# mbzuai-oryx/Video-LLaVA

Hardware: NVIDIA H100
Metric: videos/sec (100-frame CLIP encode + 7B 32-tok decode) (higher is better)
Workload: dtype bf16

## Files before the change

include/vcl.h:

```cpp
#ifndef VCL_H_
#define VCL_H_

#include <stddef.h>
#include <stdint.h>

#ifdef __cplusplus
extern "C" {
#endif

#define VCL_VERSION 1

#define VCL_DTYPE_F16 0
#define VCL_DTYPE_BF16 1

#define VCL_PIXELS_BF16_NCHW 0
#define VCL_PIXELS_U8_NHWC 1

#define VCL_WEIGHTS_BF16 0
#define VCL_WEIGHTS_FP8_E4M3 1

#define VCL_PROJ_LINEAR 0
#define VCL_PROJ_MLP2X_GELU 1

typedef struct vcl_handle vcl_handle;
// ... 110 lines not shown
#define VCL_LOGPROBS_MAX 20
int vcl_llm_set_logprobs(vcl_handle* h, int n, const int32_t* clips_host, const int32_t* top_n_host, void* stream);

int vcl_llm_read_logprobs(vcl_handle* h, int entry, int first_pos, int count, int32_t* ids_out, float* lp_out,
                          void* stream);

#define VCL_BEAM_MAX 8
typedef struct vcl_beam_record {
  float score;
  int32_t beam;
  int32_t token;
} vcl_beam_record;
int vcl_llm_beam_start(vcl_handle* h, const int64_t* ids, const void* video_feats, const int32_t* vid_start,
                       const int32_t* n_pad_host, int B, int S, int num_beams, int n_new, int eos_token,
                       void* records_out, int32_t* picks_out, void* stream);
int vcl_llm_beam_decode(vcl_handle* h, int n_steps, void* records_out, int32_t* picks_out, void* stream);

int vcl_llm_set_block_table(vcl_handle* h, const int32_t* table_host, void* stream);

int vcl_kv_block_copy(vcl_handle* h, int block, int write, void* buf, void* stream);

int vcl_llm_score(vcl_handle* h, const int64_t* ids, const void* video_feats, const int32_t* vid_start,
                  const int32_t* n_pad_host, int B, int S, const int64_t* labels, void* logits_out, float* nll_out,
                  float* loss_out, void* stream);

long long vcl_launch_count(void);

int vcl_op_gemm(const void* A, int64_t lda, const void* W, int64_t ldw, void* C, int64_t ldc,
                const void* bias, const void* residual, int64_t ldr, int M, int N, int K, int act,
                int block_n, void* stream);
int vcl_op_gemm_ex(const void* A, int64_t lda, const void* W, int64_t ldw, void* C, int64_t ldc,
                   const void* bias, const void* residual, int64_t ldr, int M, int N, int K, int act,
                   int block_n, int cluster, void* stream);
int vcl_op_cross_entropy(const void* logits, int64_t ld, const int64_t* labels, int rows, int V,
                         float* nll_out, float* loss_out, void* stream);
int vcl_op_sample(const float* logits, int64_t ld, int B, int V, const float* temperature_host,
                  const int32_t* top_k_host, const uint64_t* seed_host, const int32_t* counter_host, int32_t* tok_out,
                  void* stream);
int vcl_op_sample_logprobs(const float* logits, int64_t ld, int B, int V, const float* temperature_host,
                           const int32_t* top_k_host, const uint64_t* seed_host, const int32_t* counter_host,
                           const int32_t* top_n_host, int32_t* tok_out, int32_t* ids_out, float* lp_out,
                           void* stream);
int vcl_op_sample_ex(const float* logits, int64_t ld, int B, int V, const float* temperature_host,
                     const int32_t* top_k_host, const uint64_t* seed_host, const int32_t* counter_host,
                     const float* top_p_host, const float* repetition_penalty_host, uint32_t* token_sets,
                     const int32_t* top_n_host, int32_t* tok_out, int32_t* ids_out, float* lp_out, void* stream);
int vcl_op_beam_select(const float* logits, int64_t ld, int B, int num_beams, int V, const float* scores, int eos_token,
                       int last_step, void* records_out, int32_t* picks_out, void* stream);
int vcl_op_layernorm(const void* x, void* y, const void* w, const void* b, int rows, int D, float eps,
                     void* stream);
int vcl_op_rmsnorm(const void* x, void* y, const void* w, int rows, int D, float eps, void* stream);
int vcl_op_attention(const void* q, const void* k, const void* v, void* o, int B, int S, int H,
                     int head_dim, float scale, int causal, void* stream);
int vcl_op_attention_vit(const void* qkv, void* out, int n_frames, int S, int H, void* stream);
int vcl_kv_cache_copy(vcl_handle* h, int layer, int write, void* k, void* v, void* stream);
int vcl_op_decode_attention(const void* q, int64_t q_ld, const void* k, const void* v, void* o, int B, int H,
                            int s_max, int kv_len, const int32_t* pos_dev, const int32_t* n_pad, float scale,
                            int o_xwin, void* stream);
int vcl_op_attention_cached(const void* q, int64_t q_ld, const void* k, const void* v, void* o, int B, int H,
                            int s_max, int start_pos, int S, const int32_t* n_pad_host, void* stream);
int vcl_op_attention_packed(const void* q, int64_t q_ld, const void* k, const void* v, void* o, int H, int s_max,
                            int n_slots, int n, const int32_t* slots_host, const int32_t* start_host,
                            const int32_t* len_host, const int32_t* flash_host, const int32_t* table_host,
                            int table_row, int n_blocks, int64_t blk, void* stream);
int vcl_op_gemv(const void* x, const void* W, void* out, const void* res, const void* norm_w,
                float eps, int B, int N, int K, void* stream);
// ... 9 lines not shown
```

video-llava_b200/csrc/gemm_tc.cu:

```cuda
#include "common.cuh"
#include "kernels.h"

#include <cudaTypedefs.h>

namespace vcl {

template <int BLOCK_N>
struct GemmCfg {
  static constexpr int BLOCK_M = 128;
  static constexpr int BLOCK_K = 64;
  static constexpr int A_BYTES = BLOCK_M * BLOCK_K * 2;
  static constexpr int B_BYTES = BLOCK_N * BLOCK_K * 2;
  static constexpr int STAGE_BYTES = A_BYTES + B_BYTES;
  static constexpr int OUT_PITCH = BLOCK_N * 2 + 16;
  static constexpr int OUT_BYTES = BLOCK_M * OUT_PITCH;
  static constexpr int BAR_BYTES = 256;
  static constexpr int STAGES = (BLOCK_N == 256) ? 3 : (BLOCK_N == 128 ? 5 : 8);
  static constexpr int SMEM_BYTES = STAGES * STAGE_BYTES + BAR_BYTES + OUT_BYTES + 1024;
  static_assert((2 * STAGES + 4) * 8 <= BAR_BYTES, "barrier area");
  static_assert(SMEM_BYTES <= 227 * 1024, "shared memory");
};

__device__ __forceinline__ float act_gelu_erf(float x) {
  x = bf16r(x);
// ... 108 lines not shown
      }
    }
#pragma unroll (ACT == ACT_ROPE ? 1 : RES_INFLIGHT)
    for (int u = 0; u < RES_INFLIGHT; ++u) {
      const int r = r0 + u * RSTEP;
      if (r >= rows) break;
      const int grow = row_base + r;
      uint4 val = *reinterpret_cast<const uint4*>(stg + r * Cfg::OUT_PITCH + c * 16);
      bf16* dst = C + (long long)grow * ldc + col;
      if constexpr (ACT == ACT_ROPE) {
        const int gh = col >> 7, d = col & 127;
        const int which = gh / rp.H, head = gh - which * rp.H;
        if (which != 0) {
          int gb, col_c;
          if (rp.pack != nullptr) {
            const int2 sp = __ldg(reinterpret_cast<const int2*>(pack_row(rp.pack, grow)));
            gb = __ldg(pack_slot(rp.pack) + sp.x); col_c = sp.y;
          } else {
            gb = grow / rp.S; col_c = rp.start_pos + grow - gb * rp.S;
          }
          dst = (which == 1 ? rp.kcache : rp.vcache) + d +
                (rp.pages.table != nullptr ? kv_paged_off(rp.pages, gb, head, col_c)
                                           : (((long long)gb * rp.H + head) * rp.s_max + col_c) * 128);
        }
      } else if (RES && residual != nullptr) {
        val.x = bf16x2_add(val.x, rr[u].x); val.y = bf16x2_add(val.y, rr[u].y);
        val.z = bf16x2_add(val.z, rr[u].z); val.w = bf16x2_add(val.w, rr[u].w);
      }
      *reinterpret_cast<uint4*>(dst) = val;
    }
  }
}

template <int BLOCK_N, int ACT, int CL>
__global__ void __launch_bounds__(384, 1)
gemm_bf16_tn_kernel(const __grid_constant__ CUtensorMap tmap_a,
                    const __grid_constant__ CUtensorMap tmap_b, bf16* C, long long ldc,
                    const bf16* __restrict__ bias, const bf16* residual, long long ldr, int M,
                    int N, int K, const RopeEpilogue rope) {
  using Cfg = GemmCfg<BLOCK_N>;
  constexpr int STAGES = Cfg::STAGES;

  extern __shared__ uint8_t smem_raw[];
  const uint32_t raw_addr = smem_u32(smem_raw);
  const uint32_t pad = ((raw_addr + 1023u) & ~1023u) - raw_addr;
  uint8_t* smem = smem_raw + pad;
  const uint32_t smem_base = raw_addr + pad;

  const uint32_t bar_base = smem_base + STAGES * Cfg::STAGE_BYTES;
  auto full_bar = [&](int s) { return bar_base + 8u * s; };
  auto empty_bar = [&](int s) { return bar_base + 8u * (STAGES + s); };
  auto staged_bar = [&](int cw) { return bar_base + 8u * (2 * STAGES + cw); };
  auto drained_bar = [&](int cw) { return bar_base + 8u * (2 * STAGES + 2 + cw); };
  uint8_t* stage_out = smem + STAGES * Cfg::STAGE_BYTES + Cfg::BAR_BYTES;

  const int wg = threadIdx.x >> 7;

  if (threadIdx.x == 0) {
    tma_prefetch_desc(&tmap_a);
    tma_prefetch_desc(&tmap_b);
    for (int s = 0; s < STAGES; ++s) {
      mbar_init(full_bar(s), 1);
      mbar_init(empty_bar(s), 2 * CL);
    }
    for (int cw = 0; cw < 2; ++cw) {
      mbar_init(staged_bar(cw), 128);
      mbar_init(drained_bar(cw), STORE_THREADS);
    }
    mbar_fence_init();
  }
  __syncthreads();
  if (CL > 1) cluster_sync_all();

  const int num_m = (M + Cfg::BLOCK_M - 1) / Cfg::BLOCK_M;
  const int num_n = (N + BLOCK_N - 1) / BLOCK_N;
  const int num_k = (K + Cfg::BLOCK_K - 1) / Cfg::BLOCK_K;
  const int cta_rank = CL > 1 ? (int)cluster_ctarank() : 0;
  const int cluster_id = blockIdx.x / CL, n_clusters = gridDim.x / CL;
  const int num_tiles = ((num_m + CL - 1) / CL) * num_n;
  constexpr uint16_t MC_MASK = (uint16_t)((1u << CL) - 1u);
  constexpr int B_SLICE_ROWS = BLOCK_N / CL;

  if (wg == 0) {
    setmaxnreg_dec<56>();
    if (threadIdx.x == 0) {
      int stage = 0;
      uint32_t phase = 0;
      for (int tile = cluster_id; tile < num_tiles; tile += n_clusters) {
        const int m_blk = (tile / num_n) * CL + cta_rank, n_blk = tile % num_n;
        for (int kb = 0; kb < num_k; ++kb) {
          mbar_wait(empty_bar(stage), phase ^ 1u);
          mbar_arrive_expect_tx(full_bar(stage), Cfg::STAGE_BYTES);
          const uint32_t a_dst = smem_base + stage * Cfg::STAGE_BYTES;
          tma_load_2d(a_dst, &tmap_a, full_bar(stage), kb * Cfg::BLOCK_K, m_blk * Cfg::BLOCK_M);
          if (CL == 1) {
            tma_load_2d(a_dst + Cfg::A_BYTES, &tmap_b, full_bar(stage), kb * Cfg::BLOCK_K, n_blk * BLOCK_N);
          } else {
            tma_load_2d_mc(a_dst + Cfg::A_BYTES + cta_rank * B_SLICE_ROWS * 128, &tmap_b,
                           full_bar(stage), kb * Cfg::BLOCK_K, n_blk * BLOCK_N + cta_rank * B_SLICE_ROWS,
                           MC_MASK);
          }
          if (++stage == STAGES) { stage = 0; phase ^= 1u; }
        }
      }
    } else if (threadIdx.x >= 32) {
      const int t = threadIdx.x - 32;
      uint32_t phase = 0;
      for (int tile = cluster_id; tile < num_tiles; tile += n_clusters) {
        const int m_blk = (tile / num_n) * CL + cta_rank, n_blk = tile % num_n;
#pragma unroll 1
        for (int cw = 0; cw < 2; ++cw) {
          mbar_wait(staged_bar(cw), phase);
          gemm_epilogue_store<BLOCK_N, ACT>(stage_out + cw * 64 * Cfg::OUT_PITCH, t, m_blk * Cfg::BLOCK_M + cw * 64,
                                            n_blk, C, ldc, residual, ldr, M, N, rope);
          mbar_arrive(drained_bar(cw));
        }
        phase ^= 1u;
      }
    }
  } else {
    setmaxnreg_inc<224>();
    const int cw = wg - 1;
    const int t = threadIdx.x & 127, lane = threadIdx.x & 31, wq = t >> 5;
    uint8_t* stg = stage_out + cw * 64 * Cfg::OUT_PITCH;
    auto release = [&](int s) {
      if (t == 0) {
        if (CL == 1) {
          mbar_arrive(empty_bar(s));
        } else {
#pragma unroll
          for (int r = 0; r < CL; ++r) mbar_arrive_cluster(mapa_cluster(empty_bar(s), (uint32_t)r));
        }
      }
    };
    float acc[BLOCK_N / 2];
    int stage = 0;
    uint32_t phase = 0, out_phase = 0;
    for (int tile = cluster_id; tile < num_tiles; tile += n_clusters) {
      const int m_blk = (tile / num_n) * CL + cta_rank, n_blk = tile % num_n;
      int prev = -1;
      for (int kb = 0; kb < num_k; ++kb) {
        mbar_wait(full_bar(stage), phase);
        const uint32_t a_addr = smem_base + stage * Cfg::STAGE_BYTES;
        const uint64_t a_desc = wgmma_desc_k_sw128(a_addr + cw * 64 * 128);
        const uint64_t b_desc = wgmma_desc_k_sw128(a_addr + Cfg::A_BYTES);
        wgmma_fence();
#pragma unroll
        for (int k = 0; k < Cfg::BLOCK_K / 16; ++k) {
          wgmma_bf16<BLOCK_N>(acc, a_desc + 2u * k, b_desc + 2u * k, (kb | k) != 0 ? 1u : 0u);
        }
        wgmma_commit();
        wgmma_wait<1>();
        if (prev >= 0) release(prev);
        prev = stage;
        if (++stage == STAGES) { stage = 0; phase ^= 1u; }
      }
      wgmma_wait<0>();
      release(prev);
      wgmma_fence_regs(acc);
      if (tile != cluster_id) {
        mbar_wait(drained_bar(cw), out_phase);
        out_phase ^= 1u;
      }
      gemm_epilogue_stage<BLOCK_N, ACT>(acc, stg, lane, wq, m_blk * Cfg::BLOCK_M + cw * 64, n_blk, bias, M, N, rope);
      mbar_arrive(staged_bar(cw));
    }
  }

  __syncthreads();
  if (CL > 1) cluster_sync_all();
}

// ... 13 lines not shown
}

int make_tmap_2d(CUtensorMap* out, const void* ptr, long long rows, long long cols, long long ld,
                 int box_rows) {
  if (resolve_encode() != 0) return -2;
  cuuint64_t gdim[2] = {(cuuint64_t)cols, (cuuint64_t)rows};
  cuuint64_t gstride[1] = {(cuuint64_t)ld * 2};
  cuuint32_t box[2] = {64u, (cuuint32_t)box_rows};
  cuuint32_t estr[2] = {1u, 1u};
  CUresult r = g_encode(out, CU_TENSOR_MAP_DATA_TYPE_BFLOAT16, 2, const_cast<void*>(ptr), gdim,
                        gstride, box, estr, CU_TENSOR_MAP_INTERLEAVE_NONE,
                        CU_TENSOR_MAP_SWIZZLE_128B, CU_TENSOR_MAP_L2_PROMOTION_L2_256B,
                        CU_TENSOR_MAP_FLOAT_OOB_FILL_NONE);
  if (r != CUDA_SUCCESS) {
    set_last_error("cuTensorMapEncodeTiled failed (%d) ptr=%p rows=%lld cols=%lld ld=%lld box=%d",
                   (int)r, ptr, rows, cols, ld, box_rows);
    return -2;
  }
  return 0;
}

static int g_num_sms = 0;
int device_num_sms() {
  if (g_num_sms == 0) {
    int dev = 0;
    cudaGetDevice(&dev);
    cudaDeviceGetAttribute(&g_num_sms, cudaDevAttrMultiProcessorCount, dev);
    if (g_num_sms <= 0) g_num_sms = 132;
  }
  return g_num_sms;
}

template <int BLOCK_N, int ACT, int CL>
static int launch_one(const GemmArgs& g, cudaStream_t stream) {
  using Cfg = GemmCfg<BLOCK_N>;
  auto kern = gemm_bf16_tn_kernel<BLOCK_N, ACT, CL>;
  CUtensorMap ta, tb;
  if (make_tmap_2d(&ta, g.A, g.M, g.K, g.lda, Cfg::BLOCK_M) != 0) return -2;
  if (make_tmap_2d(&tb, g.W, g.N, g.K, g.ldw, BLOCK_N / CL) != 0) return -2;
  const int num_m = (g.M + 127) / 128;
  const int num_tiles = ((num_m + CL - 1) / CL) * ((g.N + BLOCK_N - 1) / BLOCK_N);
  cudaLaunchConfig_t cfg = {};
  cfg.blockDim = dim3(384);
  cfg.dynamicSmemBytes = Cfg::SMEM_BYTES;
  cfg.stream = stream;
  cudaLaunchAttribute attr[1];
  attr[0].id = cudaLaunchAttributeClusterDimension;
  attr[0].val.clusterDim.x = CL;
  attr[0].val.clusterDim.y = 1;
  attr[0].val.clusterDim.z = 1;
  cfg.attrs = attr;
  cfg.numAttrs = CL > 1 ? 1 : 0;
  static int resident = 0;
  if (resident == 0) {
    if (CL > 1) {
      cfg.gridDim = dim3(CL);
      VCL_CUDA_OK(cudaOccupancyMaxActiveClusters(&resident, kern, &cfg));
    }
    if (resident <= 0) resident = device_num_sms() / CL;
  }
  int clusters = resident;
  if (clusters > num_tiles) clusters = num_tiles;
  if (g.max_ctas > 0 && clusters * CL > g.max_ctas) clusters = g.max_ctas / CL > 0 ? g.max_ctas / CL : 1;
  cfg.gridDim = dim3(clusters * CL);
  VCL_CUDA_OK(cudaLaunchKernelEx(&cfg, kern, ta, tb, g.C, (long long)g.ldc, g.bias, g.residual,
                                 (long long)g.ldr, g.M, g.N, g.K, g.rope));
  count_launches(1);
  return 0;
}

template <int BLOCK_N, int ACT>
static int launch_cl(const GemmArgs& g, int cl, cudaStream_t stream) {
  if (BLOCK_N >= 128) {
    if (cl == 4) return launch_one<BLOCK_N, ACT, (BLOCK_N >= 128 ? 4 : 1)>(g, stream);
    if (cl == 2) return launch_one<BLOCK_N, ACT, (BLOCK_N >= 128 ? 2 : 1)>(g, stream);
  }
  return launch_one<BLOCK_N, ACT, 1>(g, stream);
}

template <int BLOCK_N>
static int launch_act(const GemmArgs& g, int cl, cudaStream_t stream) {
  switch (g.act) {
    case ACT_NONE: return launch_cl<BLOCK_N, ACT_NONE>(g, cl, stream);
    case ACT_QGELU: return launch_cl<BLOCK_N, ACT_QGELU>(g, cl, stream);
    case ACT_GELU: return launch_cl<BLOCK_N, ACT_GELU>(g, cl, stream);
    case ACT_SWIGLU: return launch_cl<BLOCK_N, ACT_SWIGLU>(g, cl, stream);
    case ACT_ROPE:
      if constexpr (BLOCK_N >= 128) return launch_cl<BLOCK_N, ACT_ROPE>(g, cl, stream);
      break;
  }
  set_last_error("gemm: unknown activation %d", g.act);
  return -1;
}

template <int BLOCK_N, int ACT>
static int init_one() {
  VCL_CUDA_OK(cudaFuncSetAttribute(gemm_bf16_tn_kernel<BLOCK_N, ACT, 1>,
                                   cudaFuncAttributeMaxDynamicSharedMemorySize,
                                   GemmCfg<BLOCK_N>::SMEM_BYTES));
  if (BLOCK_N >= 128) {
    VCL_CUDA_OK(cudaFuncSetAttribute(gemm_bf16_tn_kernel<BLOCK_N, ACT, (BLOCK_N >= 128 ? 2 : 1)>,
                                     cudaFuncAttributeMaxDynamicSharedMemorySize,
                                     GemmCfg<BLOCK_N>::SMEM_BYTES));
    VCL_CUDA_OK(cudaFuncSetAttribute(gemm_bf16_tn_kernel<BLOCK_N, ACT, (BLOCK_N >= 128 ? 4 : 1)>,
                                     cudaFuncAttributeMaxDynamicSharedMemorySize,
                                     GemmCfg<BLOCK_N>::SMEM_BYTES));
  }
  return 0;
}
template <int BLOCK_N>
static int init_bn() {
  if (init_one<BLOCK_N, ACT_NONE>() || init_one<BLOCK_N, ACT_QGELU>() ||
      init_one<BLOCK_N, ACT_GELU>() || init_one<BLOCK_N, ACT_SWIGLU>()) return -2;
  if constexpr (BLOCK_N >= 128) {
    if (init_one<BLOCK_N, ACT_ROPE>()) return -2;
  }
  return 0;
}
int init_gemm_kernels() {
  if (resolve_encode() != 0) return -2;
  if (init_bn<256>() || init_bn<128>() || init_bn<64>() || init_bn<32>()) return -2;
  return 0;
}

int launch_gemm_bf16_tn(const GemmArgs& g, cudaStream_t stream) {
  VCL_REQUIRE(g.M > 0 && g.N > 0 && g.K > 0, "gemm: empty problem M=%d N=%d K=%d", g.M, g.N, g.K);
  VCL_REQUIRE(g.K % 64 == 0, "gemm: K=%d must be a multiple of 64", g.K);
  VCL_REQUIRE(g.N % 32 == 0, "gemm: N=%d must be a multiple of 32", g.N);
  VCL_REQUIRE(g.lda % 8 == 0 && g.ldw % 8 == 0 && g.ldc % 8 == 0, "gemm: pitches must be x8");
  VCL_REQUIRE(((uintptr_t)g.A % 16) == 0 && ((uintptr_t)g.W % 16) == 0 &&
                  ((uintptr_t)g.C % 16) == 0, "gemm: pointers must be 16-byte aligned");
  VCL_REQUIRE(g.residual == nullptr || (g.ldr % 8 == 0 && ((uintptr_t)g.residual % 16) == 0),
              "gemm: residual must be 16-byte aligned with pitch x8");
  VCL_REQUIRE(g.bias == nullptr || ((uintptr_t)g.bias % 16) == 0, "gemm: bias alignment");
  VCL_REQUIRE(!(g.act == ACT_SWIGLU && g.residual != nullptr), "gemm: swiglu takes no residual");
  if (g.act == ACT_ROPE) {
    const RopeEpilogue& r = g.rope;
    VCL_REQUIRE(r.cos_t && r.sin_t && r.kcache && r.vcache && r.S > 0 && r.H > 0, "gemm: ACT_ROPE needs the RoPE tables and the cache");
    VCL_REQUIRE(g.N == 3 * r.H * 128 && (r.pack != nullptr || g.M % r.S == 0) && r.start_pos + r.S <= r.s_max &&
                    g.bias == nullptr && g.residual == nullptr,
                "gemm: ACT_ROPE shape (N=%d, H=%d, M=%d, S=%d, start %d, cache %d)", g.N, r.H, g.M, r.S, r.start_pos, r.s_max);
    VCL_REQUIRE(((uintptr_t)r.kcache % 16) == 0 && ((uintptr_t)r.vcache % 16) == 0 && ((uintptr_t)r.cos_t % 16) == 0 &&
                    ((uintptr_t)r.sin_t % 16) == 0, "gemm: ACT_ROPE pointers must be 16-byte aligned");
  }
  int bn = g.block_n;
  int cl = g.cluster;
  if (bn == 0) {
    const int sms = device_num_sms();
    const long long mt = (g.M + 127) / 128;
    if (mt == 1) {
      bn = 256;
      while (bn > 32 && (g.N % bn != 0 || g.N / bn < sms)) bn >>= 1;
      if (g.N % bn != 0) bn = 32;
    } else if (g.N % 256 == 0 && mt * (g.N / 256) >= sms && !(g.N <= 1024 && g.K <= 1024)) {
      bn = 256;
    } else {
      bn = (g.N % 128 == 0) ? 128 : (g.N % 64 == 0) ? 64 : 32;
    }
  }
  if (cl == 0) cl = 1;
  if (cl == -2) cl = (bn == 256 || bn == 128) && g.N % bn == 0 ? 2 : 1;
  if (g.act == ACT_ROPE && g.block_n == 0 && bn < 128) bn = 128;
  VCL_REQUIRE(g.act != ACT_ROPE || bn == 128 || bn == 256, "gemm: ACT_ROPE needs 128- or 256-wide tiles (one head = 128 columns), got %d", bn);
  VCL_REQUIRE(cl == 1 || cl == 2 || cl == 4, "gemm: cluster must be 1, 2 or 4 (got %d)", cl);
  switch (bn) {
    case 256: return launch_act<256>(g, cl, stream);
    case 128: return launch_act<128>(g, cl, stream);
    case 64: return launch_act<64>(g, 1, stream);
    case 32: return launch_act<32>(g, 1, stream);
  }
  set_last_error("gemm: unsupported block_n %d", bn);
  return -1;
}

}
```

video-llava_b200/csrc/kernels.h:

```cpp
#pragma once

#include <cuda.h>
#include <cuda_bf16.h>
#include <cuda_runtime.h>
#include <stdint.h>

namespace vcl {

typedef __nv_bfloat16 bf16;

constexpr int PACK_SEQ_MAX = 64;
constexpr int PACK_HEAD = 6 * PACK_SEQ_MAX;
inline size_t pack_elems(long long rows) { return PACK_HEAD + 2 * (size_t)rows; }
template <class T> __host__ __device__ inline T* pack_off(T* p) { return p; }
template <class T> __host__ __device__ inline T* pack_len(T* p) { return p + PACK_SEQ_MAX; }
template <class T> __host__ __device__ inline T* pack_slot(T* p) { return p + 2 * PACK_SEQ_MAX; }
template <class T> __host__ __device__ inline T* pack_last(T* p) { return p + 3 * PACK_SEQ_MAX; }
template <class T> __host__ __device__ inline T* pack_start(T* p) { return p + 4 * PACK_SEQ_MAX; }
template <class T> __host__ __device__ inline T* pack_end(T* p) { return p + 5 * PACK_SEQ_MAX; }
template <class T> __host__ __device__ inline T* pack_row(T* p, long long r) { return p + PACK_HEAD + 2 * r; }

struct KvPages {
  const int* table = nullptr;
  int row = 0;
// ... 3 lines not shown
  return (long long)__ldg(p.table + slot * p.row + (col >> 7)) * p.blk + ((long long)head * 128 + (col & 127)) * 128;
}

enum Act { ACT_NONE = 0, ACT_QGELU = 1, ACT_GELU = 2, ACT_SWIGLU = 3, ACT_ROPE = 4 };
struct RopeEpilogue {
  const bf16* cos_t = nullptr; const bf16* sin_t = nullptr;
  bf16* kcache = nullptr; bf16* vcache = nullptr;
  int S = 0, start_pos = 0, H = 0, s_max = 0;
  const int* n_pad = nullptr;
  const int* pack = nullptr;
  KvPages pages;
};


void set_last_error(const char* fmt, ...);
void count_launches(long long n);
long long launch_count();
int device_num_sms();

struct GemmArgs {
  const bf16* A = nullptr;  long long lda = 0;
  const bf16* W = nullptr;  long long ldw = 0;
  bf16* C = nullptr;        long long ldc = 0;
  const bf16* bias = nullptr;
  const bf16* residual = nullptr; long long ldr = 0;
  int M = 0, N = 0, K = 0;
  int act = ACT_NONE;
  int block_n = 0;
  int cluster = 0;
  int max_ctas = 0;
  RopeEpilogue rope;
};
int launch_gemm_bf16_tn(const GemmArgs& g, cudaStream_t stream);
int init_gemm_kernels();
int make_tmap_2d(CUtensorMap* out, const void* ptr, long long rows, long long cols, long long ld,
                 int box_rows);

int launch_layernorm(const bf16* x, long long ldx, bf16* y, long long ldy, const bf16* w,
                     const bf16* b, int rows, int D, float eps, cudaStream_t stream);
int launch_rmsnorm(const bf16* x, long long ldx, bf16* y, long long ldy, const bf16* w, int rows,
                   int D, float eps, cudaStream_t stream);
int launch_im2col(const void* pixels, int mode, bf16* out, int n_frames, int image, int patch,
                  int KP, cudaStream_t stream);
int launch_clip_embed_ln(const bf16* patch_out, const bf16* cls, const bf16* pos, const bf16* ln_w,
                         const bf16* ln_b, bf16* h, int n_frames, int P, int D, float eps,
                         cudaStream_t stream);
int launch_embed_splice(const long long* ids, const bf16* table, const bf16* vid, const int* vid_start,
                        bf16* h, int B, int S, int D, int n_vid, int vocab, cudaStream_t stream,
                        const int* pack = nullptr, int M = 0);
int launch_rope_table(bf16* cos_t, bf16* sin_t, int max_pos, int head_dim, float theta,
                      cudaStream_t stream);
int launch_rope_kv_prefill(bf16* qkv, bf16* kcache, bf16* vcache, const bf16* cos_t,
                           const bf16* sin_t, int B, int S, int H, int head_dim, int s_max, int pos0,
                           cudaStream_t stream, const int* pos_dev = nullptr, const int* n_pad = nullptr);
int launch_embed_tokens(const int* tok, long long tok_stride, const bf16* table, bf16* h, int B,
                        int D, int vocab, cudaStream_t stream);
int launch_argmax(const float* logits, int* out, long long out_stride, int B, int V,
                  cudaStream_t stream);
int launch_fill_int(int* dst, int value, int n, cudaStream_t stream);

int launch_st_pool(const void* feats, int in_dtype, long long frame_stride, long long patch_stride,
                   int T, int P, int C, int n_temporal, void* out, int out_dtype,
                   cudaStream_t stream);

int launch_cross_entropy(const bf16* logits, long long ld, int V, const long long* labels, long long row0, int rows,
                         int seg, float* nll, bf16* logits_out, cudaStream_t stream);
// ... 126 lines not shown
```

video-llava_b200/csrc/vcl_api.cu:

```cuda
#include "../../include/vcl.h"

#include <stdarg.h>
#include <stdio.h>
#include <stdlib.h>
#include <string.h>

#include <algorithm>
#include <map>
#include <string>
#include <vector>

#include "common.cuh"
#include "kernels.h"

namespace vcl {

static thread_local char g_err[1024] = "";
static long long g_launches = 0;

void count_launches(long long n) { g_launches += n; }
long long launch_count() { return g_launches; }

void set_last_error(const char* fmt, ...) {
  va_list ap;
// ... 1563 lines not shown
int vcl_kv_block_copy(vcl_handle* h, int block, int write, void* buf, void* stream) {
  VCL_REQUIRE(h && buf, "vcl_kv_block_copy: null argument");
  VCL_REQUIRE(h->paged(), "vcl_kv_block_copy: the handle has a contiguous KV cache (kv_blocks 0)");
  VCL_REQUIRE(block >= 0 && block < h->cfg.kv_blocks, "vcl_kv_block_copy: block %d outside 0..%d", block,
              h->cfg.kv_blocks - 1);
  bf16* blk = h->pool + (size_t)block * h->block_elems();
  const size_t bytes = h->block_elems() * sizeof(bf16);
  cudaStream_t st = as_stream(stream);
  if (write) VCL_CUDA_OK(cudaMemcpyAsync(blk, buf, bytes, cudaMemcpyDefault, st));
  else VCL_CUDA_OK(cudaMemcpyAsync(buf, blk, bytes, cudaMemcpyDefault, st));
  return 0;
}

int vcl_op_gemm(const void* A, int64_t lda, const void* W, int64_t ldw, void* C, int64_t ldc,
                const void* bias, const void* residual, int64_t ldr, int M, int N, int K, int act,
                int block_n, void* stream) {
  return vcl_op_gemm_ex(A, lda, W, ldw, C, ldc, bias, residual, ldr, M, N, K, act, block_n, 0, stream);
}

int vcl_op_gemm_ex(const void* A, int64_t lda, const void* W, int64_t ldw, void* C, int64_t ldc,
                   const void* bias, const void* residual, int64_t ldr, int M, int N, int K, int act,
                   int block_n, int cluster, void* stream) {
  if (check_device() != 0) return -2;
  static bool inited = false;
  if (!inited) {
    VCL_TRY(init_gemm_kernels());
    inited = true;
  }
  return gemm(reinterpret_cast<const bf16*>(A), lda, reinterpret_cast<const bf16*>(W), ldw,
              reinterpret_cast<bf16*>(C), ldc, reinterpret_cast<const bf16*>(bias),
              reinterpret_cast<const bf16*>(residual), ldr, M, N, K, act, as_stream(stream), block_n, cluster);
}

int vcl_op_cross_entropy(const void* logits, int64_t ld, const int64_t* labels, int rows, int V, float* nll_out,
                         float* loss_out, void* stream) {
  if (check_device() != 0) return -2;
  VCL_REQUIRE(logits != nullptr && labels != nullptr && nll_out != nullptr,
              "vcl_op_cross_entropy: logits, labels and nll_out are required");
  const long long* lab = reinterpret_cast<const long long*>(labels);
  VCL_TRY(launch_cross_entropy(reinterpret_cast<const bf16*>(logits), ld, V, lab, 0, rows, 0, nll_out, nullptr,
                               as_stream(stream)));
  return loss_out != nullptr ? launch_nll_mean(nll_out, lab, rows, 0, nullptr, loss_out, as_stream(stream)) : 0;
}

}

namespace {

int op_sample(const char* name, const float* logits, int64_t ld, int B, int V, const float* temperature_host,
              const int32_t* top_k_host, const uint64_t* seed_host, const int32_t* counter_host,
              const int32_t* top_n_host, int32_t* tok_out, int32_t* ids_out, float* lp_out, void* stream,
              const float* top_p_host = nullptr, const float* rep_host = nullptr, uint32_t* tset = nullptr) {
  if (check_device() != 0) return -2;
  VCL_REQUIRE(logits && temperature_host && top_k_host && seed_host && counter_host && tok_out, "%s: null argument",
              name);
  VCL_REQUIRE(B >= 1, "%s: B=%d", name, B);
  const bool wide = top_p_host != nullptr;
  if (wide) {
    VCL_REQUIRE(rep_host != nullptr, "%s: null argument", name);
    VCL_REQUIRE(V >= 1 && V <= VCL_SAMPLE_WIDE_MAX_V, "%s: V=%d outside 1..%d (the 32-bit sampler's shared memory)",
                name, V, VCL_SAMPLE_WIDE_MAX_V);
    for (int b = 0; b < B; ++b)
      VCL_REQUIRE(top_p_host[b] >= 0.f && top_p_host[b] <= 1.f && isfinite(rep_host[b]) && rep_host[b] > 0.f,
                  "%s: row %d: top_p %g outside [0, 1] or repetition_penalty %g not a finite value > 0", name, b,
                  (double)top_p_host[b], (double)rep_host[b]);
  }
// ... 366 lines not shown
```

video-llava_b200/vcl_native.py:

```python
from __future__ import annotations

import ctypes
import operator
import os
from ctypes import POINTER, Structure, c_char_p, c_float, c_int, c_int32, c_int64, c_uint64, c_void_p

import torch

_HERE = os.path.dirname(os.path.abspath(__file__))
LIB_PATH = os.path.join(_HERE, "libvcl.so")

DTYPE_F16, DTYPE_BF16 = 0, 1
PIXELS_BF16_NCHW, PIXELS_U8_NHWC = 0, 1
PROJ_LINEAR, PROJ_MLP2X_GELU = 0, 1
NO_VIDEO = -2 ** 31
ACT_NONE, ACT_QGELU, ACT_GELU, ACT_SWIGLU = 0, 1, 2, 3
WEIGHTS_BF16, WEIGHTS_FP8_E4M3 = 0, 1
WEIGHT_FORMATS = {"bf16": WEIGHTS_BF16, "fp8_e4m3": WEIGHTS_FP8_E4M3}


def weight_format_code(name) -> int:
    if not isinstance(name, str) or name not in WEIGHT_FORMATS:
        raise ValueError(f"unknown LLM weight format {name!r}: one of {sorted(WEIGHT_FORMATS)}")
    return WEIGHT_FORMATS[name]


class VclError(RuntimeError):
    pass


class vcl_config(Structure):
    _fields_ = [
        ("clip_layers", c_int32), ("clip_hidden", c_int32), ("clip_inter", c_int32),
        ("clip_heads", c_int32), ("image_size", c_int32), ("patch_size", c_int32),
        ("clip_ln_eps", c_float),
        ("llm_layers", c_int32), ("llm_hidden", c_int32), ("llm_inter", c_int32),
        ("llm_heads", c_int32), ("vocab", c_int32), ("rms_eps", c_float), ("rope_theta", c_float),
        ("proj_type", c_int32), ("n_temporal", c_int32),
        ("max_frames", c_int32), ("max_batch", c_int32), ("max_seq", c_int32),
        ("max_slots", c_int32),
    ]


class vcl_config_ex(vcl_config):
    _fields_ = [("kv_blocks", c_int32)]


KV_BLOCK_COLS = 128

# ... 62 lines not shown
                                      c_void_p, c_void_p, c_void_p]),
    "vcl_llm_slots_prefill_chunk": (c_int, [c_void_p, c_int, POINTER(c_int32), POINTER(c_int32), POINTER(c_int32),
                                            POINTER(c_int32), c_void_p, c_void_p, c_void_p, c_void_p, c_void_p]),
    "vcl_llm_slots_prefill_append": (c_int, [c_void_p, c_int, POINTER(c_int32), POINTER(c_int32), POINTER(c_int32),
                                             c_void_p, c_void_p, c_void_p]),
    "vcl_llm_slot_decode": (c_int, [c_void_p, c_void_p, POINTER(c_int32), c_int, c_int, c_void_p, c_void_p]),
    "vcl_llm_set_sampling": (c_int, [c_void_p, c_int, POINTER(c_int32), POINTER(c_float), POINTER(c_int32),
                                     POINTER(c_uint64), c_void_p]),
    "vcl_llm_set_sampling_ex": (c_int, [c_void_p, c_int, POINTER(c_int32), POINTER(c_float), POINTER(c_int32),
                                        POINTER(c_uint64), POINTER(c_float), POINTER(c_float), c_void_p]),
    "vcl_llm_set_token_set": (c_int, [c_void_p, c_int, c_void_p, c_int, c_void_p]),
    "vcl_llm_read_token_set": (c_int, [c_void_p, c_int, c_void_p, c_void_p]),
    "vcl_llm_set_logprobs": (c_int, [c_void_p, c_int, POINTER(c_int32), POINTER(c_int32), c_void_p]),
    "vcl_llm_read_logprobs": (c_int, [c_void_p, c_int, c_int, c_int, c_void_p, c_void_p, c_void_p]),
    "vcl_llm_beam_start": (c_int, [c_void_p, c_void_p, c_void_p, c_void_p, POINTER(c_int32), c_int, c_int, c_int, c_int,
                                   c_int, c_void_p, c_void_p, c_void_p]),
    "vcl_llm_beam_decode": (c_int, [c_void_p, c_int, c_void_p, c_void_p, c_void_p]),
    "vcl_launch_count": (ctypes.c_longlong, []),
    "vcl_kv_cache_copy": (c_int, [c_void_p, c_int, c_int, c_void_p, c_void_p, c_void_p]),
    "vcl_llm_set_block_table": (c_int, [c_void_p, POINTER(c_int32), c_void_p]),
    "vcl_kv_block_copy": (c_int, [c_void_p, c_int, c_int, c_void_p, c_void_p]),
    "vcl_op_decode_attention": (c_int, [c_void_p, c_int64, c_void_p, c_void_p, c_void_p, c_int, c_int, c_int, c_int,
                                        c_void_p, c_void_p, c_float, c_int, c_void_p]),
    "vcl_op_attention_cached": (c_int, [c_void_p, c_int64, c_void_p, c_void_p, c_void_p, c_int, c_int, c_int, c_int,
                                        c_int, POINTER(c_int32), c_void_p]),
    "vcl_op_attention_packed": (c_int, [c_void_p, c_int64, c_void_p, c_void_p, c_void_p, c_int, c_int, c_int, c_int,
                                        POINTER(c_int32), POINTER(c_int32), POINTER(c_int32), POINTER(c_int32),
                                        POINTER(c_int32), c_int, c_int, c_int64, c_void_p]),
    "vcl_op_cross_entropy": (c_int, [c_void_p, c_int64, c_void_p, c_int, c_int, c_void_p, c_void_p, c_void_p]),
    "vcl_op_gemm": (c_int, [c_void_p, c_int64, c_void_p, c_int64, c_void_p, c_int64, c_void_p, c_void_p,
                            c_int64, c_int, c_int, c_int, c_int, c_int, c_void_p]),
    "vcl_op_gemm_ex": (c_int, [c_void_p, c_int64, c_void_p, c_int64, c_void_p, c_int64, c_void_p, c_void_p,
                               c_int64, c_int, c_int, c_int, c_int, c_int, c_int, c_void_p]),
    "vcl_op_sample": (c_int, [c_void_p, c_int64, c_int, c_int, POINTER(c_float), POINTER(c_int32), POINTER(c_uint64),
                              POINTER(c_int32), c_void_p, c_void_p]),
    "vcl_op_sample_logprobs": (c_int, [c_void_p, c_int64, c_int, c_int, POINTER(c_float), POINTER(c_int32),
                                       POINTER(c_uint64), POINTER(c_int32), POINTER(c_int32), c_void_p, c_void_p,
                                       c_void_p, c_void_p]),
    "vcl_op_sample_ex": (c_int, [c_void_p, c_int64, c_int, c_int, POINTER(c_float), POINTER(c_int32), POINTER(c_uint64),
                                 POINTER(c_int32), POINTER(c_float), POINTER(c_float), c_void_p, POINTER(c_int32),
                                 c_void_p, c_void_p, c_void_p, c_void_p]),
    "vcl_op_beam_select": (c_int, [c_void_p, c_int64, c_int, c_int, c_int, c_void_p, c_int, c_int, c_void_p, c_void_p,
                                   c_void_p]),
    "vcl_op_layernorm": (c_int, [c_void_p, c_void_p, c_void_p, c_void_p, c_int, c_int, c_float, c_void_p]),
    "vcl_op_rmsnorm": (c_int, [c_void_p, c_void_p, c_void_p, c_int, c_int, c_float, c_void_p]),
    "vcl_op_attention": (c_int, [c_void_p, c_void_p, c_void_p, c_void_p, c_int, c_int, c_int, c_int,
                                 c_float, c_int, c_void_p]),
    "vcl_op_attention_vit": (c_int, [c_void_p, c_void_p, c_int, c_int, c_int, c_void_p]),
    "vcl_op_gemv": (c_int, [c_void_p, c_void_p, c_void_p, c_void_p, c_void_p, c_float, c_int, c_int,
                            c_int, c_void_p]),
    "vcl_op_gemv_fp8": (c_int, [c_void_p, c_void_p, c_void_p, c_void_p, c_void_p, c_float, c_int, c_int,
                                c_int, c_void_p]),
    "vcl_op_quantize_fp8": (c_int, [c_void_p, c_int, c_int, c_void_p, c_void_p, c_void_p, c_void_p]),
}

EXPORTED_SYMBOLS = tuple(_SIGNATURES)

_lib = None


def lib() -> ctypes.CDLL:
    global _lib
    if _lib is None:
        if not os.path.exists(LIB_PATH):
            raise VclError(f"{LIB_PATH} is missing: run `python video-llava_b200/build.py` "
                           "(there is no CPU or PyTorch fallback for this path)")
# ... 20 lines not shown

def cur_stream() -> c_void_p:
    return c_void_p(torch.cuda.current_stream().cuda_stream)


def _dtype_code(dt: torch.dtype) -> int:
    if dt == torch.float16:
        return DTYPE_F16
    if dt == torch.bfloat16:
        return DTYPE_BF16
    raise VclError(f"unsupported dtype {dt} (fp16 / bf16 only)")


def st_pool(features: torch.Tensor, n_temporal: int = 100, out_dtype: torch.dtype = torch.float16):
    T, P, C = features.shape
    assert features.is_cuda and features.stride(2) == 1
    out = torch.empty(n_temporal + P, C, dtype=out_dtype, device=features.device)
    check(lib().vcl_st_pool(c_void_p(features.data_ptr()), _dtype_code(features.dtype),
                            features.stride(0), features.stride(1), T, P, C, n_temporal,
                            ptr(out), _dtype_code(out_dtype), cur_stream()))
    return out


def op_gemm(a, w, bias=None, residual=None, act=ACT_NONE, block_n=0, out=None, cluster=0):
    M, K = a.shape
    N = w.shape[0]
    n_out = N // 2 if act == ACT_SWIGLU else N
    if out is None:
        out = torch.empty(M, n_out, dtype=torch.bfloat16, device=a.device)
    check(lib().vcl_op_gemm_ex(ptr(a), a.stride(0), ptr(w), w.stride(0), ptr(out), out.stride(0), ptr(bias),
                               ptr(residual), residual.stride(0) if residual is not None else 0, M, N, K,
                               act, block_n, cluster, cur_stream()))
    return out


def op_layernorm(x, w, b, eps):
    y = torch.empty_like(x)
    check(lib().vcl_op_layernorm(ptr(x), ptr(y), ptr(w), ptr(b), x.shape[0], x.shape[1], eps, cur_stream()))
    return y


def op_rmsnorm(x, w, eps):
    y = torch.empty_like(x)
    check(lib().vcl_op_rmsnorm(ptr(x), ptr(y), ptr(w), x.shape[0], x.shape[1], eps, cur_stream()))
    return y


def op_attention(q, k, v, scale, causal):
    B, S, H, hd = q.shape
    o = torch.empty_like(q)
    check(lib().vcl_op_attention(ptr(q), ptr(k), ptr(v), ptr(o), B, S, H, hd, scale, int(causal), cur_stream()))
    return o


def op_attention_vit(qkv, n_frames, S, H):
    out = torch.empty(n_frames * S, H * 64, dtype=torch.bfloat16, device=qkv.device)
    check(lib().vcl_op_attention_vit(ptr(qkv), ptr(out), n_frames, S, H, cur_stream()))
    return out


def op_cross_entropy(logits, labels, V=None, want_loss=True):
    rows, ld = logits.shape
    assert logits.dtype == torch.bfloat16 and logits.stride(1) == 1
    lab = labels.to(device=logits.device, dtype=torch.int64).contiguous()
    nll = torch.empty(rows, dtype=torch.float32, device=logits.device)
    loss = torch.empty((), dtype=torch.float32, device=logits.device) if want_loss else None
# ... 573 lines not shown
```

Measured before the change: 5.118.

## Split GEMM wave-quantization tail into narrower-tile second launch; add weight-major tile order

Adds a tile-region abstraction so a GEMM can be run as a head region with the normal tile width plus a tail region with narrower tiles. The tail covers the partial last wave, so the final wave finishes sooner when the tile count is not a multiple of the SM count. It also adds an N-major tile traversal for small-M GEMMs whose activations fit in L2, so each weight tile is reused across consecutive M tiles. The cost is an extra kernel launch, more templated dispatch, and a new schedule-query API.

New measurement: 5.238, median of 6. 1.02x the previous value.

```diff
diff --git a/include/vcl.h b/include/vcl.h
--- a/include/vcl.h
+++ b/include/vcl.h
@@ -166,6 +166,7 @@
 int vcl_op_gemm_ex(const void* A, int64_t lda, const void* W, int64_t ldw, void* C, int64_t ldc,
                    const void* bias, const void* residual, int64_t ldr, int M, int N, int K, int act,
                    int block_n, int cluster, void* stream);
+int vcl_gemm_schedule(int M, int N, int K, int act, int* out);
 int vcl_op_cross_entropy(const void* logits, int64_t ld, const int64_t* labels, int rows, int V,
                          float* nll_out, float* loss_out, void* stream);
 int vcl_op_sample(const float* logits, int64_t ld, int B, int V, const float* temperature_host,
diff --git a/video-llava_b200/csrc/gemm_tc.cu b/video-llava_b200/csrc/gemm_tc.cu
--- a/video-llava_b200/csrc/gemm_tc.cu
+++ b/video-llava_b200/csrc/gemm_tc.cu
@@ -164,12 +164,27 @@
   }
 }
 
+struct TileRegion {
+  int m0, n0, num_m, num_n;
+  int n_major;
+};
+
+template <int CL>
+__device__ __forceinline__ void region_tile(const TileRegion& rg, int tile, int cta_rank, int& m_blk, int& n_blk) {
+  const bool n_major = CL == 1 && rg.n_major;
+  const int num_mg = (rg.num_m + CL - 1) / CL;
+  const int mi = n_major ? tile % num_mg : tile / rg.num_n;
+  const int ni = n_major ? tile / num_mg : tile % rg.num_n;
+  m_blk = rg.m0 + mi * CL + cta_rank;
+  n_blk = rg.n0 + ni;
+}
+
 template <int BLOCK_N, int ACT, int CL>
 __global__ void __launch_bounds__(384, 1)
 gemm_bf16_tn_kernel(const __grid_constant__ CUtensorMap tmap_a,
                     const __grid_constant__ CUtensorMap tmap_b, bf16* C, long long ldc,
                     const bf16* __restrict__ bias, const bf16* residual, long long ldr, int M,
-                    int N, int K, const RopeEpilogue rope) {
+                    int N, int K, const TileRegion rg, const RopeEpilogue rope) {
   using Cfg = GemmCfg<BLOCK_N>;
   constexpr int STAGES = Cfg::STAGES;
 
@@ -204,12 +219,11 @@
   __syncthreads();
   if (CL > 1) cluster_sync_all();
 
-  const int num_m = (M + Cfg::BLOCK_M - 1) / Cfg::BLOCK_M;
-  const int num_n = (N + BLOCK_N - 1) / BLOCK_N;
+  const int num_n = rg.num_n;
   const int num_k = (K + Cfg::BLOCK_K - 1) / Cfg::BLOCK_K;
   const int cta_rank = CL > 1 ? (int)cluster_ctarank() : 0;
   const int cluster_id = blockIdx.x / CL, n_clusters = gridDim.x / CL;
-  const int num_tiles = ((num_m + CL - 1) / CL) * num_n;
+  const int num_tiles = ((rg.num_m + CL - 1) / CL) * num_n;
   constexpr uint16_t MC_MASK = (uint16_t)((1u << CL) - 1u);
   constexpr int B_SLICE_ROWS = BLOCK_N / CL;
 
@@ -219,7 +233,8 @@
       int stage = 0;
       uint32_t phase = 0;
       for (int tile = cluster_id; tile < num_tiles; tile += n_clusters) {
-        const int m_blk = (tile / num_n) * CL + cta_rank, n_blk = tile % num_n;
+        int m_blk, n_blk;
+      region_tile<CL>(rg, tile, cta_rank, m_blk, n_blk);
         for (int kb = 0; kb < num_k; ++kb) {
           mbar_wait(empty_bar(stage), phase ^ 1u);
           mbar_arrive_expect_tx(full_bar(stage), Cfg::STAGE_BYTES);
@@ -239,7 +254,8 @@
       const int t = threadIdx.x - 32;
       uint32_t phase = 0;
       for (int tile = cluster_id; tile < num_tiles; tile += n_clusters) {
-        const int m_blk = (tile / num_n) * CL + cta_rank, n_blk = tile % num_n;
+        int m_blk, n_blk;
+        region_tile<CL>(rg, tile, cta_rank, m_blk, n_blk);
 #pragma unroll 1
         for (int cw = 0; cw < 2; ++cw) {
           mbar_wait(staged_bar(cw), phase);
@@ -269,7 +285,8 @@
     int stage = 0;
     uint32_t phase = 0, out_phase = 0;
     for (int tile = cluster_id; tile < num_tiles; tile += n_clusters) {
-      const int m_blk = (tile / num_n) * CL + cta_rank, n_blk = tile % num_n;
+      int m_blk, n_blk;
+        region_tile<CL>(rg, tile, cta_rank, m_blk, n_blk);
       int prev = -1;
       for (int kb = 0; kb < num_k; ++kb) {
         mbar_wait(full_bar(stage), phase);
@@ -349,14 +366,13 @@
 }
 
 template <int BLOCK_N, int ACT, int CL>
-static int launch_one(const GemmArgs& g, cudaStream_t stream) {
+static int launch_one(const GemmArgs& g, const TileRegion& rg, cudaStream_t stream) {
   using Cfg = GemmCfg<BLOCK_N>;
   auto kern = gemm_bf16_tn_kernel<BLOCK_N, ACT, CL>;
   CUtensorMap ta, tb;
   if (make_tmap_2d(&ta, g.A, g.M, g.K, g.lda, Cfg::BLOCK_M) != 0) return -2;
   if (make_tmap_2d(&tb, g.W, g.N, g.K, g.ldw, BLOCK_N / CL) != 0) return -2;
-  const int num_m = (g.M + 127) / 128;
-  const int num_tiles = ((num_m + CL - 1) / CL) * ((g.N + BLOCK_N - 1) / BLOCK_N);
+  const int num_tiles = ((rg.num_m + CL - 1) / CL) * rg.num_n;
   cudaLaunchConfig_t cfg = {};
   cfg.blockDim = dim3(384);
   cfg.dynamicSmemBytes = Cfg::SMEM_BYTES;
@@ -381,33 +397,81 @@
   if (g.max_ctas > 0 && clusters * CL > g.max_ctas) clusters = g.max_ctas / CL > 0 ? g.max_ctas / CL : 1;
   cfg.gridDim = dim3(clusters * CL);
   VCL_CUDA_OK(cudaLaunchKernelEx(&cfg, kern, ta, tb, g.C, (long long)g.ldc, g.bias, g.residual,
-                                 (long long)g.ldr, g.M, g.N, g.K, g.rope));
+                                 (long long)g.ldr, g.M, g.N, g.K, rg, g.rope));
   count_launches(1);
   return 0;
 }
 
 template <int BLOCK_N, int ACT>
-static int launch_cl(const GemmArgs& g, int cl, cudaStream_t stream) {
+static int launch_cl(const GemmArgs& g, const TileRegion& rg, int cl, cudaStream_t stream) {
   if (BLOCK_N >= 128) {
-    if (cl == 4) return launch_one<BLOCK_N, ACT, (BLOCK_N >= 128 ? 4 : 1)>(g, stream);
-    if (cl == 2) return launch_one<BLOCK_N, ACT, (BLOCK_N >= 128 ? 2 : 1)>(g, stream);
-  }
-  return launch_one<BLOCK_N, ACT, 1>(g, stream);
+    if (cl == 4) return launch_one<BLOCK_N, ACT, (BLOCK_N >= 128 ? 4 : 1)>(g, rg, stream);
+    if (cl == 2) return launch_one<BLOCK_N, ACT, (BLOCK_N >= 128 ? 2 : 1)>(g, rg, stream);
+  }
+  return launch_one<BLOCK_N, ACT, 1>(g, rg, stream);
 }
 
 template <int BLOCK_N>
-static int launch_act(const GemmArgs& g, int cl, cudaStream_t stream) {
+static int launch_act(const GemmArgs& g, const TileRegion& rg, int cl, cudaStream_t stream) {
   switch (g.act) {
-    case ACT_NONE: return launch_cl<BLOCK_N, ACT_NONE>(g, cl, stream);
-    case ACT_QGELU: return launch_cl<BLOCK_N, ACT_QGELU>(g, cl, stream);
-    case ACT_GELU: return launch_cl<BLOCK_N, ACT_GELU>(g, cl, stream);
-    case ACT_SWIGLU: return launch_cl<BLOCK_N, ACT_SWIGLU>(g, cl, stream);
+    case ACT_NONE: return launch_cl<BLOCK_N, ACT_NONE>(g, rg, cl, stream);
+    case ACT_QGELU: return launch_cl<BLOCK_N, ACT_QGELU>(g, rg, cl, stream);
+    case ACT_GELU: return launch_cl<BLOCK_N, ACT_GELU>(g, rg, cl, stream);
+    case ACT_SWIGLU: return launch_cl<BLOCK_N, ACT_SWIGLU>(g, rg, cl, stream);
     case ACT_ROPE:
-      if constexpr (BLOCK_N >= 128) return launch_cl<BLOCK_N, ACT_ROPE>(g, cl, stream);
+      if constexpr (BLOCK_N >= 128) return launch_cl<BLOCK_N, ACT_ROPE>(g, rg, cl, stream);
       break;
   }
   set_last_error("gemm: unknown activation %d", g.act);
   return -1;
+}
+
+static bool one_width() {
+  const char* e = getenv("VCL_GEMM_ONE_WIDTH");
+  return e != nullptr && e[0] != '\0' && e[0] != '0';
+}
+
+static int launch_bn(const GemmArgs& g, int bn, const TileRegion& rg, int cl, cudaStream_t stream) {
+  switch (bn) {
+    case 256: return launch_act<256>(g, rg, cl, stream);
+    case 128: return launch_act<128>(g, rg, cl, stream);
+    case 64: return launch_act<64>(g, rg, 1, stream);
+    case 32: return launch_act<32>(g, rg, 1, stream);
+  }
+  set_last_error("gemm: unsupported block_n %d", bn);
+  return -1;
+}
+
+struct TailPlan {
+  TileRegion head, tail;
+  int w = 0;
+};
+static TailPlan plan_tail(int M, int N, int K, int bn, int act, int slots) {
+  TailPlan best;
+  const int num_m = (M + 127) / 128, num_n = (N + bn - 1) / bn;
+  const long long T = (long long)num_m * num_n;
+  const long long full = T / slots * slots;
+  if (K < 2048 || full == 0 || T == full || 4 * (T - full) >= 3LL * slots) return best;
+  auto rounds = [&](long long tiles) { return (tiles + slots - 1) / slots; };
+  long long best_cost = rounds(T) * bn;
+  for (int cut = 0; cut < 2; ++cut) {
+    const int h = cut == 0 ? (int)(full / num_n) : (int)(full / num_m);
+    if (h == 0 || h == (cut == 0 ? num_m : num_n)) continue;
+    const TileRegion head = cut == 0 ? TileRegion{0, 0, h, num_n} : TileRegion{0, 0, num_m, h};
+    for (int w = bn / 2; w >= bn / 4; w /= 2) {
+      if (w < 64 || (act == ACT_ROPE && w < 128)) break;
+      const TileRegion tail = cut == 0 ? TileRegion{h, 0, num_m - h, (N + w - 1) / w}
+                                       : TileRegion{0, h * (bn / w), num_m, (N - h * bn + w - 1) / w};
+      if (rounds((long long)tail.num_m * tail.num_n) > 1) continue;
+      const long long cost = rounds((long long)head.num_m * head.num_n) * bn +
+                             rounds((long long)tail.num_m * tail.num_n) * w;
+      if (cost < best_cost) {
+        best_cost = cost;
+        best.head = head; best.tail = tail; best.w = w;
+      }
+    }
+  }
+  return best;
 }
 
 template <int BLOCK_N, int ACT>
@@ -438,6 +502,37 @@
   if (resolve_encode() != 0) return -2;
   if (init_bn<256>() || init_bn<128>() || init_bn<64>() || init_bn<32>()) return -2;
   return 0;
+}
+
+static int auto_block_n(int M, int N, int K, int act) {
+  const int sms = device_num_sms();
+  const long long mt = (M + 127) / 128;
+  int bn;
+  if (mt == 1) {
+    bn = 256;
+    while (bn > 32 && (N % bn != 0 || N / bn < sms)) bn >>= 1;
+    if (N % bn != 0) bn = 32;
+  } else if (N % 256 == 0 && mt * (N / 256) >= sms && !(N <= 1024 && K <= 1024)) {
+    bn = 256;
+  } else {
+    bn = (N % 128 == 0) ? 128 : (N % 64 == 0) ? 64 : 32;
+  }
+  if (act == ACT_ROPE && bn < 128) bn = 128;
+  return bn;
+}
+
+static int l2_bytes() {
+  static int bytes = 0;
+  if (bytes == 0) {
+    int dev = 0;
+    cudaGetDevice(&dev);
+    cudaDeviceGetAttribute(&bytes, cudaDevAttrL2CacheSize, dev);
+    if (bytes <= 0) bytes = 50 * 1024 * 1024;
+  }
+  return bytes;
+}
+static int weight_major(int M, int N, int K) {
+  return M < N && 2LL * M * K <= l2_bytes() / 4 ? 1 : 0;
 }
 
 int launch_gemm_bf16_tn(const GemmArgs& g, cudaStream_t stream) {
@@ -460,34 +555,34 @@
     VCL_REQUIRE(((uintptr_t)r.kcache % 16) == 0 && ((uintptr_t)r.vcache % 16) == 0 && ((uintptr_t)r.cos_t % 16) == 0 &&
                     ((uintptr_t)r.sin_t % 16) == 0, "gemm: ACT_ROPE pointers must be 16-byte aligned");
   }
-  int bn = g.block_n;
+  int bn = g.block_n != 0 ? g.block_n : auto_block_n(g.M, g.N, g.K, g.act);
   int cl = g.cluster;
-  if (bn == 0) {
-    const int sms = device_num_sms();
-    const long long mt = (g.M + 127) / 128;
-    if (mt == 1) {
-      bn = 256;
-      while (bn > 32 && (g.N % bn != 0 || g.N / bn < sms)) bn >>= 1;
-      if (g.N % bn != 0) bn = 32;
-    } else if (g.N % 256 == 0 && mt * (g.N / 256) >= sms && !(g.N <= 1024 && g.K <= 1024)) {
-      bn = 256;
-    } else {
-      bn = (g.N % 128 == 0) ? 128 : (g.N % 64 == 0) ? 64 : 32;
-    }
-  }
   if (cl == 0) cl = 1;
   if (cl == -2) cl = (bn == 256 || bn == 128) && g.N % bn == 0 ? 2 : 1;
-  if (g.act == ACT_ROPE && g.block_n == 0 && bn < 128) bn = 128;
   VCL_REQUIRE(g.act != ACT_ROPE || bn == 128 || bn == 256, "gemm: ACT_ROPE needs 128- or 256-wide tiles (one head = 128 columns), got %d", bn);
   VCL_REQUIRE(cl == 1 || cl == 2 || cl == 4, "gemm: cluster must be 1, 2 or 4 (got %d)", cl);
-  switch (bn) {
-    case 256: return launch_act<256>(g, cl, stream);
-    case 128: return launch_act<128>(g, cl, stream);
-    case 64: return launch_act<64>(g, 1, stream);
-    case 32: return launch_act<32>(g, 1, stream);
-  }
-  set_last_error("gemm: unsupported block_n %d", bn);
-  return -1;
-}
-
-}
+  const int n_major = weight_major(g.M, g.N, g.K);
+  if (g.block_n == 0 && cl == 1 && !one_width()) {
+    const int sms = device_num_sms();
+    TailPlan p = plan_tail(g.M, g.N, g.K, bn, g.act, g.max_ctas > 0 && g.max_ctas < sms ? g.max_ctas : sms);
+    if (p.w != 0) {
+      p.head.n_major = p.tail.n_major = n_major;
+      if (const int e = launch_bn(g, bn, p.head, 1, stream)) return e;
+      return launch_bn(g, p.w, p.tail, 1, stream);
+    }
+  }
+  return launch_bn(g, bn, TileRegion{0, 0, (g.M + 127) / 128, (g.N + bn - 1) / bn, cl == 1 ? n_major : 0}, cl, stream);
+}
+
+int gemm_schedule(int M, int N, int K, int act, int out[4]) {
+  VCL_REQUIRE(M > 0 && N > 0 && K > 0 && N % 32 == 0, "gemm_schedule: shape M=%d N=%d K=%d", M, N, K);
+  const int bn = auto_block_n(M, N, K, act);
+  const TailPlan p = one_width() ? TailPlan{} : plan_tail(M, N, K, bn, act, device_num_sms());
+  out[0] = bn;
+  out[1] = p.w != 0 ? p.head.num_m * p.head.num_n : ((M + 127) / 128) * ((N + bn - 1) / bn);
+  out[2] = p.w;
+  out[3] = p.w != 0 ? p.tail.num_m * p.tail.num_n : 0;
+  return 0;
+}
+
+}
diff --git a/video-llava_b200/csrc/kernels.h b/video-llava_b200/csrc/kernels.h
--- a/video-llava_b200/csrc/kernels.h
+++ b/video-llava_b200/csrc/kernels.h
@@ -59,6 +59,7 @@
   RopeEpilogue rope;
 };
 int launch_gemm_bf16_tn(const GemmArgs& g, cudaStream_t stream);
+int gemm_schedule(int M, int N, int K, int act, int out[4]);
 int init_gemm_kernels();
 int make_tmap_2d(CUtensorMap* out, const void* ptr, long long rows, long long cols, long long ld,
                  int box_rows);
diff --git a/video-llava_b200/csrc/vcl_api.cu b/video-llava_b200/csrc/vcl_api.cu
--- a/video-llava_b200/csrc/vcl_api.cu
+++ b/video-llava_b200/csrc/vcl_api.cu
@@ -1619,6 +1619,12 @@
               reinterpret_cast<const bf16*>(residual), ldr, M, N, K, act, as_stream(stream), block_n, cluster);
 }
 
+int vcl_gemm_schedule(int M, int N, int K, int act, int* out) {
+  if (check_device() != 0) return -2;
+  VCL_REQUIRE(out != nullptr, "vcl_gemm_schedule: out is null");
+  return gemm_schedule(M, N, K, act, out);
+}
+
 int vcl_op_cross_entropy(const void* logits, int64_t ld, const int64_t* labels, int rows, int V, float* nll_out,
                          float* loss_out, void* stream) {
   if (check_device() != 0) return -2;
diff --git a/video-llava_b200/vcl_native.py b/video-llava_b200/vcl_native.py
--- a/video-llava_b200/vcl_native.py
+++ b/video-llava_b200/vcl_native.py
@@ -15,6 +15,7 @@
 PROJ_LINEAR, PROJ_MLP2X_GELU = 0, 1
 NO_VIDEO = -2 ** 31
 ACT_NONE, ACT_QGELU, ACT_GELU, ACT_SWIGLU = 0, 1, 2, 3
+ACT_ROPE = 4
 WEIGHTS_BF16, WEIGHTS_FP8_E4M3 = 0, 1
 WEIGHT_FORMATS = {"bf16": WEIGHTS_BF16, "fp8_e4m3": WEIGHTS_FP8_E4M3}
 
@@ -143,6 +144,7 @@
                             c_int64, c_int, c_int, c_int, c_int, c_int, c_void_p]),
     "vcl_op_gemm_ex": (c_int, [c_void_p, c_int64, c_void_p, c_int64, c_void_p, c_int64, c_void_p, c_void_p,
                                c_int64, c_int, c_int, c_int, c_int, c_int, c_int, c_void_p]),
+    "vcl_gemm_schedule": (c_int, [c_int, c_int, c_int, c_int, POINTER(c_int32)]),
     "vcl_op_sample": (c_int, [c_void_p, c_int64, c_int, c_int, POINTER(c_float), POINTER(c_int32), POINTER(c_uint64),
                               POINTER(c_int32), c_void_p, c_void_p]),
     "vcl_op_sample_logprobs": (c_int, [c_void_p, c_int64, c_int, c_int, POINTER(c_float), POINTER(c_int32),
@@ -229,6 +231,12 @@
                                ptr(residual), residual.stride(0) if residual is not None else 0, M, N, K,
                                act, block_n, cluster, cur_stream()))
     return out
+
+
+def gemm_schedule(M, N, K, act=ACT_NONE):
+    out = (c_int32 * 4)()
+    check(lib().vcl_gemm_schedule(M, N, K, act, out))
+    return tuple(out)
 
 
 def op_layernorm(x, w, b, eps):
```
